# fankiat/sopht-mpi

Measured on NVIDIA B200. Metric: full_timestep_Mcell_updates_per_s, higher is better.
Workload: dtype f32

## Files before the change

sopht_mpi_b200/csrc/poisson_fft.cu:

```cuda
#include "fft_device.h"
#include "poisson.h"

#include <cstdlib>
#include <vector>

#define SB_P32_LINES(log2n) 8


#ifndef SB200_EMU
#define SB_DEV_ALLOC(ptr, bytes) (cudaMalloc((void**)&(ptr), (bytes)) == cudaSuccess)
#define SB_DEV_FREE(ptr) cudaFree(ptr)
#define SB_DEV_UPLOAD(dst, src, bytes, stream) \
  cudaMemcpyAsync(dst, src, bytes, cudaMemcpyHostToDevice, (cudaStream_t)(stream))
#define SB_STREAM_SYNC(stream) cudaStreamSynchronize((cudaStream_t)(stream))
#else
#define SB_DEV_ALLOC(ptr, bytes) (((ptr) = (decltype(ptr))malloc(bytes)) != nullptr)
#define SB_DEV_FREE(ptr) free(ptr)
#define SB_DEV_UPLOAD(dst, src, bytes, stream) memcpy(dst, src, bytes)
#define SB_STREAM_SYNC(stream) (void)0
#endif

struct SbLines {
  int inner, n1, n2;
  long long s1, s2;
  long long pt;
  int o1_shift = 30;
  long long s1_hi = 0;
  int gsh = 31;
  long long s_grp = 0;
  int rot = 0;
  SB_HD long long base(int i, int o1, int o2) const {
    return ((i + ((o1 >> 1) & rot)) & ((1u << gsh) - 1)) + (long long)(i >> gsh) * s_grp +
           (long long)(o1 & ((1 << o1_shift) - 1)) * s1 + (long long)(o1 >> o1_shift) * s1_hi + o2 * s2;
  }
};

template <typename T>
struct FieldRows {
  T* f;
  int ny, gs, dim;
  long long my, mx, vol;
  SB_D T* row(int c, int z, int y) const {
    return f + (dim == 3 ? c * vol + ((long long)(z + gs) * my + (y + gs)) * mx + gs
                         : c * vol + (long long)(y + gs) * mx + gs);
  }
  SB_D C2<T> load(int c, int z, int y, int m) const {
    const T* p = row(c, z, y) + 2 * m;
    if ((gs & 1) == 0) return *reinterpret_cast<const C2<T>*>(p);
    return C2<T>{p[0], p[1]};
  }
};
template <typename T>
struct GreensRows {
  SbGreens<T> g;
  int ny;
  SB_D C2<T> load(int, int z, int y, int m) const { return C2<T>{g(z, y, 2 * m), g(z, y, 2 * m + 1)}; }
};

static inline int sb_slab_kxl(int nx, int nranks) { return ((nx + 1 + nranks - 1) / nranks + 3) & ~3; }

struct SbRowBlocks {
  int kxl = 0;
  unsigned magic = 0;
  long long dblk = 0;
  SB_D long long rel(int k) const {
#ifdef SB200_EMU
    const int b = k / kxl;
#else
    const int b = (int)__umulhi((unsigned)k, magic);
#endif
    return (long long)b * dblk + k;
  }
  SB_D long long row(long long line, long long pitch) const { return line * (kxl ? (long long)kxl : pitch); }
};
static inline SbRowBlocks sb_row_blocks(int kxl, long long blk) {
  SbRowBlocks rb;
  rb.kxl = kxl;
  rb.magic = kxl ? (unsigned)((0x100000000ULL + (unsigned long long)kxl - 1) / (unsigned long long)kxl) : 0;
  rb.dblk = blk - kxl;
  return rb;
}

template <typename T, typename Rows, bool PRUNED, int LOG2N, int LINES>
__global__ void __launch_bounds__(LOG2N > 0 ? LINES * (1 << LOG2N) / SB_FFT_R : 512)
    sb_fft_x_r2c_kernel(SbFftPlan plan, int lines_rt, Rows rows, C2<T>* out, long long out_pitch,
                        const C2<T>* __restrict__ tw, const C2<T>* __restrict__ wpost, SbRowBlocks rb) {
  SB_DYN_SMEM(smem_raw);
  C2<T>* sm = reinterpret_cast<C2<T>*>(smem_raw);
  const int Tn = LOG2N > 0 ? (1 << LOG2N) / SB_FFT_R : plan.threads, N = LOG2N > 0 ? (1 << LOG2N) : plan.n;
  const int lines_per_block = LOG2N > 0 ? LINES : lines_rt;
  const int l = threadIdx.x / Tn, t = threadIdx.x - l * Tn;
  const int y = blockIdx.x * lines_per_block + l;
  const int z = blockIdx.y, c = blockIdx.z;
  const bool valid = y < rows.ny;
  const int yc = valid ? y : rows.ny - 1;
  const SbSmemLine<T, false> sl = sb_smem_line<T, false>(sm, l, 0, sb_fft_npad(N));
  constexpr int IN = PRUNED ? SB_FFT_R / 2 : SB_FFT_R;
  C2<T> v[SB_FFT_R];
#pragma unroll
  for (int p = 0; p < SB_FFT_R; ++p) v[p] = p < IN ? rows.load(c, z, yc, t + p * Tn) : C2<T>{T(0), T(0)};
  if constexpr (LOG2N > 0)
    sb_fft_forward_c<T, LOG2N, false, LINES>(v, t, tw, SbFftLineC<T, LOG2N, false, LINES>::line(sm, l));
  else
    sb_fft_forward<T, false>(v, plan, t, tw, sl);
#pragma unroll
  for (int p = 0; p < SB_FFT_R; ++p) sl.at(t + p * Tn) = v[p];
  __syncthreads();
  if (valid) {
    const long long line = ((long long)c * gridDim.y + z) * rows.ny + y;
    C2<T>* row = out + rb.row(line, out_pitch);
    C2<T> r[SB_FFT_R];
#pragma unroll
    for (int p = 0; p < SB_FFT_R; ++p) {
      const int k = t + p * Tn;
      const C2<T> zk = v[p];
      const C2<T> zc = cconj(sl.at((N - k) & (N - 1)));
      const C2<T> wd = cmul(wpost[k], csub(zk, zc));
      const C2<T> s = cadd(zk, zc);
      r[p] = C2<T>{T(0.5) * (s.x + wd.y), T(0.5) * (s.y - wd.x)};
    }
    const C2<T> last{v[0].x - v[0].y, T(0)};
    if (rb.kxl == 0) {
#pragma unroll
      for (int p = 0; p < SB_FFT_R; ++p) row[t + p * Tn] = r[p];
      if (t == 0) row[N] = last;
    } else {
#pragma unroll
      for (int p = 0; p < SB_FFT_R; ++p) row[rb.rel(t + p * Tn)] = r[p];
      if (t == 0) row[rb.rel(N)] = last;
    }
  }
}

template <typename T, int LOG2N, int LINES>
__global__ void __launch_bounds__(LOG2N > 0 ? LINES * (1 << LOG2N) / SB_FFT_R : 512)
    sb_fft_x_c2r_kernel(SbFftPlan plan, int lines_rt, const C2<T>* in, long long in_pitch,
                        FieldRows<T> rows, const C2<T>* __restrict__ tw, const C2<T>* __restrict__ wpost,
                        SbRowBlocks rb) {
  SB_DYN_SMEM(smem_raw);
  C2<T>* sm = reinterpret_cast<C2<T>*>(smem_raw);
  const int Tn = LOG2N > 0 ? (1 << LOG2N) / SB_FFT_R : plan.threads, N = LOG2N > 0 ? (1 << LOG2N) : plan.n;
  const int lines_per_block = LOG2N > 0 ? LINES : lines_rt;
  const int l = threadIdx.x / Tn, t = threadIdx.x - l * Tn;
  const int y = blockIdx.x * lines_per_block + l;
  const int z = blockIdx.y, c = blockIdx.z;
  const bool valid = y < rows.ny;
  const int yc = valid ? y : rows.ny - 1;
  const SbSmemLine<T, false> sl = sb_smem_line<T, false>(sm, l, 0, sb_fft_npad(N));
  const long long line = ((long long)c * gridDim.y + z) * rows.ny + yc;
  const C2<T>* row = in + rb.row(line, in_pitch);
  C2<T> v[SB_FFT_R];
  if (rb.kxl == 0) {
#pragma unroll
    for (int p = 0; p < SB_FFT_R; ++p) v[p] = row[t + p * Tn];
    if (t == 0) sl.at(N) = row[N];
  } else {
#pragma unroll
    for (int p = 0; p < SB_FFT_R; ++p) v[p] = row[rb.rel(t + p * Tn)];
    if (t == 0) sl.at(N) = row[rb.rel(N)];
  }
#pragma unroll
  for (int p = 0; p < SB_FFT_R; ++p) sl.at(t + p * Tn) = v[p];
  __syncthreads();
#pragma unroll
  for (int p = 0; p < SB_FFT_R; ++p) {
    const int k = t + p * Tn;
    const C2<T> xk = sl.at(k);
    const C2<T> xc = cconj(sl.at(N - k));
    const C2<T> wd = cmul(cconj(wpost[k]), csub(xk, xc));
    const C2<T> s = cadd(xk, xc);
    v[p] = C2<T>{s.x - wd.y, s.y + wd.x};
  }
  __syncthreads();
  if constexpr (LOG2N > 0)
    sb_fft_inverse_c<T, LOG2N, false, LINES>(v, t, tw, SbFftLineC<T, LOG2N, false, LINES>::line(sm, l));
  else
    sb_fft_inverse<T, false>(v, plan, t, tw, sl);
  if (valid) {
    T* orow = rows.row(c, z, y);
#pragma unroll
    for (int p = 0; p < SB_FFT_R / 2; ++p) {
      const int m = t + p * Tn;
      if ((rows.gs & 1) == 0) {
        *reinterpret_cast<C2<T>*>(orow + 2 * m) = v[p];
      } else {
        orow[2 * m] = v[p].x;
        orow[2 * m + 1] = v[p].y;
      }
    }
  }
}

constexpr int sb_lb_threads(int log2n, int lines) { return log2n > 0 ? lines * ((1 << log2n) / SB_FFT_R) : 512; }
constexpr int sb_lb_blocks(int log2n, int lines, size_t elem) {
  return (log2n > 0 && elem == 4) ? 1024 / sb_lb_threads(log2n, lines) : 1;
}

constexpr int sb_lb_blocks_conv(int log2n, int lines, size_t elem) {
  if (!(log2n > 0 && elem == 4)) return 1;
  const int nt = sb_lb_threads(log2n, lines);
  return nt <= 256 ? 768 / nt : nt <= 512 ? 1024 / nt : 1;
}

template <typename T>
struct SbGreensTable {
  const T* g;
  long long g_pt, g_s1;
  int n1_full = 1;
  int o1_off = 0;
  const T* g2 = nullptr;
  int kx0 = 0, kx_last = 1 << 30;
};

SB_D void sb_cp_async16(void* smem_dst, const void* gsrc) {
#ifdef SB200_EMU
  memcpy(smem_dst, gsrc, 16);
#else
  asm volatile("cp.async.cg.shared.global [%0], [%1], 16;" ::"r"((unsigned)__cvta_generic_to_shared(smem_dst)),
               "l"(gsrc)
               : "memory");
#endif
}
SB_D void sb_cp_async_wait_all() {
#ifndef SB200_EMU
  asm volatile("cp.async.wait_all;" ::: "memory");
#endif
}

template <typename T, int MODE, int LOG2N, int LINES, bool G2>
__global__ void __launch_bounds__(sb_lb_threads(LOG2N, LINES), MODE == 1 ? sb_lb_blocks_conv(LOG2N, LINES, sizeof(T)) : sb_lb_blocks(LOG2N, LINES, sizeof(T)))
    sb_fft_strided_kernel(SbFftPlan plan, int lb_shift_rt, const C2<T>* in, SbLines lin, C2<T>* out, SbLines lout,
                          const C2<T>* __restrict__ tw, SbGreensTable<T> gt) {
  SB_DYN_SMEM(smem_raw);
  C2<T>* sm = reinterpret_cast<C2<T>*>(smem_raw);
  const int Tn = LOG2N > 0 ? (1 << LOG2N) / SB_FFT_R : plan.threads, n = LOG2N > 0 ? (1 << LOG2N) : plan.n;
  constexpr int LINES_SHIFT = LINES == 16 ? 4 : LINES == 8 ? 3 : LINES == 4 ? 2 : LINES == 2 ? 1 : 0;
  const int lb_shift = LOG2N > 0 ? LINES_SHIFT : lb_shift_rt;
  const int l = threadIdx.x & ((1 << lb_shift) - 1), t = threadIdx.x >> lb_shift;
  static_assert(!G2 || (MODE == 1 && LOG2N > 0 && sizeof(T) == 4), "thread-order table: fused float kernel");
  const int ib = G2 ? blockIdx.y : blockIdx.x;
  const int i = (ib << lb_shift) + l;
  const int o1 = G2 ? blockIdx.z : blockIdx.y, o2 = G2 ? blockIdx.x : blockIdx.z;
  const bool valid = i < lin.inner;
  const int ic = valid ? i : lin.inner - 1;
  const SbSmemLine<T, true> sl = sb_smem_line<T, true>(sm, l, lb_shift, sb_fft_npad(n));
  float4* gstage = nullptr;
  if constexpr (G2) {
    constexpr int NT = LINES * ((1 << LOG2N) / SB_FFT_R);
    gstage = reinterpret_cast<float4*>(sm + LINES * SbFftC<LOG2N>::npad) + threadIdx.x;
    const int g1 = o1 + gt.o1_off;
    const int m1 = g1 <= (gt.n1_full >> 1) ? g1 : gt.n1_full - g1;
    const float4* src = reinterpret_cast<const float4*>(gt.g2) +
                        (((long long)m1 * gridDim.y + ib) * NT + threadIdx.x) * 4;
#pragma unroll
    for (int k = 0; k < 4; ++k) sb_cp_async16(gstage + k * NT, src + k);
  }
  constexpr int IN = (MODE == 0 || MODE == 1) ? SB_FFT_R / 2 : SB_FFT_R;
  constexpr int OUT = (MODE == 1 || MODE == 2) ? SB_FFT_R / 2 : SB_FFT_R;
  C2<T> v[SB_FFT_R];
  {
    const C2<T>* gp = in + lin.base(ic, o1, o2);
    const long long sp = (long long)Tn * lin.pt;
    gp += (long long)t * lin.pt;
#pragma unroll
    for (int p = 0; p < SB_FFT_R; ++p) {
      if (p < IN) {
        v[p] = *gp;
        gp += sp;
      } else {
        v[p] = C2<T>{T(0), T(0)};
      }
    }
  }
  if constexpr (MODE != 2) {
    if constexpr (LOG2N > 0)
      sb_fft_forward_c<T, LOG2N, true, LINES>(v, t, tw, SbFftLineC<T, LOG2N, true, LINES>::line(sm, l));
    else
      sb_fft_forward<T, true>(v, plan, t, tw, sl);
  }
  if constexpr (G2) {
    constexpr int NT = LINES * ((1 << LOG2N) / SB_FFT_R);
    sb_cp_async_wait_all();
#pragma unroll
    for (int k = 0; k < 4; ++k) {
      const float4 gv = gstage[k * NT];
      v[4 * k] = cscale(v[4 * k], gv.x);
      v[4 * k + 1] = cscale(v[4 * k + 1], gv.y);
      v[4 * k + 2] = cscale(v[4 * k + 2], gv.z);
      v[4 * k + 3] = cscale(v[4 * k + 3], gv.w);
    }
  } else if constexpr (MODE == 1) {
    const int g1 = o1 + gt.o1_off;
    const int m1 = g1 <= (gt.n1_full >> 1) ? g1 : gt.n1_full - g1;
    const int kxg = ic + gt.kx0 < gt.kx_last ? ic + gt.kx0 : gt.kx_last;
    const T* g = gt.g + ((long long)m1 * gt.g_s1 + kxg);
    const long long gs = (long long)Tn * gt.g_pt;
    const T* ga = g + (long long)t * gt.g_pt;
    const T* gb = g + (long long)(n - t - (SB_FFT_R / 2) * Tn) * gt.g_pt;
#pragma unroll
    for (int p = 0; p < SB_FFT_R / 2; ++p) {
      v[p] = cscale(v[p], *ga);
      v[p + SB_FFT_R / 2] = cscale(v[p + SB_FFT_R / 2], *gb);
      ga += gs;
      gb -= gs;
    }
  }
  if constexpr (MODE == 1 || MODE == 2) {
    if constexpr (LOG2N > 0)
      sb_fft_inverse_c<T, LOG2N, true, LINES>(v, t, tw, SbFftLineC<T, LOG2N, true, LINES>::line(sm, l));
    else
      sb_fft_inverse<T, true>(v, plan, t, tw, sl);
  }
  if (valid) {
    C2<T>* gp = out + lout.base(i, o1, o2);
    const long long sp = (long long)Tn * lout.pt;
    gp += (long long)t * lout.pt;
#pragma unroll
    for (int p = 0; p < OUT; ++p) {
      *gp = v[p];
      gp += sp;
    }
  }
}

constexpr int sb_p32_min_blocks(int log2n, int lines) {
  const int nt = lines * ((1 << log2n) / SB_FFT_P32);
  return 512 / nt > 0 ? 512 / nt : 1;
}

template <typename T, int MODE, int LOG2N, int LINES>
__global__ void __launch_bounds__(LINES*((1 << LOG2N) / SB_FFT_P32), sb_p32_min_blocks(LOG2N, LINES))
    sb_fft_strided32_kernel(const C2<T>* in, SbLines lin, C2<T>* out, SbLines lout,
                            const C2<T>* __restrict__ tw, SbGreensTable<T> gt) {
  SB_DYN_SMEM(smem_raw);
  using FC = SbFft32C<LOG2N>;
  constexpr int PT = SB_FFT_P32, Tn = FC::Tn;
  constexpr int LINES_SHIFT = LINES == 16 ? 4 : LINES == 8 ? 3 : LINES == 4 ? 2 : LINES == 2 ? 1 : 0;
  constexpr int IN = (MODE == 0 || MODE == 1) ? PT / 2 : PT;
  constexpr int OUT = (MODE == 1 || MODE == 2) ? PT / 2 : PT;
  C2<T>* sm = reinterpret_cast<C2<T>*>(smem_raw);
  const int l = threadIdx.x & (LINES - 1), t = threadIdx.x >> LINES_SHIFT;
  const int i = (blockIdx.x << LINES_SHIFT) + l;
  const int o1 = blockIdx.y, o2 = blockIdx.z;
  const bool valid = i < lin.inner;
  const int ic = valid ? i : lin.inner - 1;
  C2<T>* sline = sm + l;
  C2<T> v[PT];
  {
    const C2<T>* gp = in + lin.base(ic, o1, o2);
    const long long sp = (long long)Tn * lin.pt;
    gp += (long long)t * lin.pt;
#pragma unroll
    for (int p = 0; p < PT; ++p) {
      if (p < IN) {
        v[p] = *gp;
        gp += sp;
      } else {
        v[p] = C2<T>{T(0), T(0)};
      }
    }
  }
  if constexpr (MODE != 2) sb_fft32_forward_c<T, LOG2N, LINES, MODE == 1>(v, t, tw, sline);
  if constexpr (MODE == 1) {
    const int g1 = o1 + gt.o1_off;
    const int m1 = g1 <= (gt.n1_full >> 1) ? g1 : gt.n1_full - g1;
    const int kxg = ic + gt.kx0 < gt.kx_last ? ic + gt.kx0 : gt.kx_last;
    const T* g = gt.g + ((long long)m1 * gt.g_s1 + kxg);
    const long long gs = (long long)Tn * gt.g_pt;
    const T* ga = g + (long long)t * gt.g_pt;
    const T* gb = g + (long long)(FC::n - t - (PT / 2) * Tn) * gt.g_pt;
#pragma unroll
    for (int p = 0; p < PT / 2; ++p) {
      v[p] = cscale(v[p], *ga);
      v[p + PT / 2] = cscale(v[p + PT / 2], *gb);
      ga += gs;
      gb -= gs;
    }
  }
  if constexpr (MODE == 1 || MODE == 2) sb_fft32_inverse_c<T, LOG2N, LINES, false>(v, t, tw, sline);
  if (valid) {
    C2<T>* gp = out + lout.base(i, o1, o2);
    const long long sp = (long long)Tn * lout.pt;
    gp += (long long)t * lout.pt;
#pragma unroll
    for (int p = 0; p < OUT; ++p) {
      *gp = v[p];
      gp += sp;
    }
  }
}

#ifndef SB200_EMU
SB_D unsigned sb_smem_u32(const void* p) { return (unsigned)__cvta_generic_to_shared(p); }
SB_D void sb_mbar_init(unsigned long long* bar, unsigned count) {
  asm volatile("mbarrier.init.shared::cta.b64 [%0], %1;" ::"r"(sb_smem_u32(bar)), "r"(count) : "memory");
  asm volatile("fence.mbarrier_init.release.cluster;" ::: "memory");
}
SB_D void sb_bulk_load(void* smem_dst, const void* gsrc, unsigned bytes, unsigned long long* bar) {
  asm volatile("fence.proxy.async.shared::cta;" ::: "memory");
  asm volatile("mbarrier.arrive.expect_tx.shared::cta.b64 _, [%0], %1;" ::"r"(sb_smem_u32(bar)), "r"(bytes)
               : "memory");
  asm volatile("cp.async.bulk.shared::cluster.global.mbarrier::complete_tx::bytes [%0], [%1], %2, [%3];" ::"r"(
                   sb_smem_u32(smem_dst)),
               "l"(gsrc), "r"(bytes), "r"(sb_smem_u32(bar))
               : "memory");
}
SB_D void sb_mbar_wait_warp(unsigned long long* bar, unsigned parity) {
  unsigned ok;
  do {
    asm volatile(
        "{\n.reg .pred p;\nmbarrier.try_wait.parity.shared::cta.b64 p, [%1], %2;\nselp.u32 %0, 1, 0, p;\n}"
        : "=r"(ok)
        : "r"(sb_smem_u32(bar)), "r"(parity)
        : "memory");
  } while (!__all_sync(0xffffffffu, ok));
}
SB_D void sb_mbar_expect_if(bool pred, unsigned long long* bar, unsigned bytes) {
  asm volatile(
      "{\n.reg .pred p;\nsetp.ne.u32 p, %0, 0;\n"
      "@p fence.proxy.async.shared::cta;\n"
      "@p mbarrier.arrive.expect_tx.shared::cta.b64 _, [%2], %1;\n}" ::"r"((unsigned)pred),
      "r"(bytes), "r"(sb_smem_u32(bar))
      : "memory");
}
SB_D void sb_bulk_copy_if(bool pred, void* smem_dst, const void* gsrc, unsigned bytes, unsigned long long* bar) {
  asm volatile(
      "{\n.reg .pred p;\nsetp.ne.u32 p, %0, 0;\n"
      "@p cp.async.bulk.shared::cluster.global.mbarrier::complete_tx::bytes [%1], [%2], %3, [%4];\n}" ::"r"(
          (unsigned)pred),
      "r"(sb_smem_u32(smem_dst)), "l"(gsrc), "r"(bytes), "r"(sb_smem_u32(bar))
      : "memory");
}
SB_D void sb_mbar_arrive(unsigned long long* bar) {
  asm volatile("mbarrier.arrive.shared::cta.b64 _, [%0];" ::"r"(sb_smem_u32(bar)) : "memory");
}
SB_D void sb_fence_async_smem() { asm volatile("fence.proxy.async.shared::cta;" ::: "memory"); }
SB_D void sb_bulk_store(void* gdst, const void* smem_src, unsigned bytes) {
  asm volatile("cp.async.bulk.global.shared::cta.bulk_group [%0], [%1], %2;" ::"l"(gdst), "r"(sb_smem_u32(smem_src)),
               "r"(bytes)
               : "memory");
  asm volatile("cp.async.bulk.commit_group;" ::: "memory");
}
SB_D void sb_bulk_wait_read() { asm volatile("cp.async.bulk.wait_group.read 0;" ::: "memory"); }
SB_D void sb_bulk_wait_all() { asm volatile("cp.async.bulk.wait_group 0;" ::: "memory"); }
#else
SB_D void sb_mbar_init(unsigned long long* bar, unsigned count) {
  __atomic_store_n(bar, ((unsigned long long)count << 8) | count, __ATOMIC_SEQ_CST);
}
SB_D void sb_mbar_update(unsigned long long* bar, unsigned arrivals, long long tx16) {
  unsigned long long e = __atomic_load_n(bar, __ATOMIC_SEQ_CST);
  for (;;) {
    const unsigned long long cnt = (e >> 8) & 0xffu, pend = (e & 0xffu) - arrivals;
    const unsigned long long tx = (unsigned long long)((long long)((e >> 16) & 0xffffu) + tx16) & 0xffffu;
    unsigned long long d = (e & 0xffffffff00000000ULL) | (tx << 16) | (cnt << 8) | pend;
    if (pend == 0 && tx == 0) d = (((e >> 32) + 1) << 32) | (cnt << 8) | cnt;
    if (__atomic_compare_exchange_n(bar, &e, d, false, __ATOMIC_SEQ_CST, __ATOMIC_SEQ_CST)) return;
  }
}
SB_D void sb_mbar_arrive(unsigned long long* bar) { sb_mbar_update(bar, 1, 0); }
SB_D void sb_mbar_expect_if(bool pred, unsigned long long* bar, unsigned bytes) {
  if (pred) sb_mbar_update(bar, 1, bytes / 16);
}
SB_D void sb_bulk_copy_if(bool pred, void* smem_dst, const void* gsrc, unsigned bytes, unsigned long long* bar) {
  if (!pred) return;
  memcpy(smem_dst, gsrc, bytes);
  sb_mbar_update(bar, 0, -(long long)(bytes / 16));
}
SB_D void sb_bulk_load(void* smem_dst, const void* gsrc, unsigned bytes, unsigned long long* bar) {
  sb_mbar_expect_if(true, bar, bytes);
  sb_bulk_copy_if(true, smem_dst, gsrc, bytes, bar);
}
SB_D void sb_mbar_wait_warp(unsigned long long* bar, unsigned parity) {
  while (((__atomic_load_n(bar, __ATOMIC_SEQ_CST) >> 32) & 1u) == parity) std::this_thread::yield();
}
SB_D void sb_fence_async_smem() { __atomic_thread_fence(__ATOMIC_SEQ_CST); }
SB_D void sb_bulk_store(void* gdst, const void* smem_src, unsigned bytes) { memcpy(gdst, smem_src, bytes); }
SB_D void sb_bulk_wait_read() {}
SB_D void sb_bulk_wait_all() {}
#endif

template <int LOG2N>
struct SbZw {
  using FC = SbFft32C<LOG2N>;
  static constexpr int Tn = FC::Tn, LINES = 8, NT = LINES * Tn, NW = NT / 32, NZ = FC::n / 2;
  static constexpr unsigned TILE = NZ * LINES;
  static constexpr int XL = SbFft32W<LOG2N>::XL;
  static constexpr int BLOCKS = LOG2N >= 10 ? 2 : 4;
  static constexpr size_t smem = 2 * TILE * sizeof(C2<float>) + (size_t)LINES * XL * sizeof(float) + 128;
  static_assert((2 + NW) * 8 + 2 * 4 + 2 * 4 <= 128, "barriers, arrival counters, tile ids");
};

template <int LOG2N>
__global__ void __launch_bounds__(SbZw<LOG2N>::NT, SbZw<LOG2N>::BLOCKS)
    sb_fft_zconvw_kernel(C2<float>* B, int ntiles, int ncomp, int ng, int nky, const C2<float>* __restrict__ tw,
                         const float* __restrict__ g5, int n1_full, int* next_tile) {
  using Z = SbZw<LOG2N>;
  constexpr int PT = SB_FFT_P32, Tn = Z::Tn, N = Z::FC::n;
  constexpr unsigned TILE = Z::TILE, TILE_BYTES = TILE * sizeof(C2<float>);
  SB_DYN_SMEM(smem_raw);
  C2<float>* tbuf = reinterpret_cast<C2<float>*>(smem_raw);
  float* xch = reinterpret_cast<float*>(tbuf + 2 * TILE);
  unsigned long long* bars = reinterpret_cast<unsigned long long*>(xch + Z::LINES * Z::XL);
  unsigned* cnt = reinterpret_cast<unsigned*>(bars + 2 + Z::NW);
  int* tile_of = reinterpret_cast<int*>(cnt + 2);
  const int tid = threadIdx.x, l = tid / Tn, t = tid % Tn, lane = tid & 31, warp = tid >> 5;
  float* xl = xch + l * Z::XL;
  const int slot = (l + (t >> 1)) & 7;
  auto tile_offset = [&](int tile) {
    const int c = tile % ncomp, r = tile / ncomp;
    return (((long long)c * ng + r % ng) * nky + r / ng) * (long long)TILE;
  };
  auto arm = [&](int b) {
    const int tile = atomicAdd(next_tile, 1);
    tile_of[b] = tile;
    if (tile < ntiles)
      sb_bulk_load(tbuf + b * TILE, B + tile_offset(tile), TILE_BYTES, bars + b);
    else
      sb_mbar_arrive(bars + b);
  };
  if (tid == 0) {
    sb_mbar_init(bars + 0, 1);
    sb_mbar_init(bars + 1, 1);
    for (int w = 0; w < Z::NW; ++w) sb_mbar_init(bars + 2 + w, 1);
    cnt[0] = cnt[1] = 0;
  }
  __syncthreads();
  if (tid == 0) {
    arm(0);
    arm(1);
  }
  for (int k = 0;; ++k) {
    const int b = k & 1;
    C2<float>* tb = tbuf + b * TILE + slot;
    sb_mbar_wait_warp(bars + b, (unsigned)(k >> 1) & 1u);
    if (tile_of[b] >= ntiles) break;
    C2<float> v[PT];
#pragma unroll
    for (int p = 0; p < PT / 2; ++p) v[p] = tb[(t + p * Tn) * Z::LINES];
    sb_fft32w_forward<LOG2N, true>(v, t, tw, xl);
    __syncwarp();
    {
      const int r = tile_of[b] / ncomp, kxg = r % ng, ky = r / ng;
      const int m1 = ky <= (n1_full >> 1) ? ky : n1_full - ky;
      constexpr int LW = 32 / Tn;
      const float* src = g5 + (((long long)m1 * ng + kxg) * Z::LINES + warp * LW) * N;
      sb_mbar_expect_if(lane == 0, bars + 2 + warp, LW * N * sizeof(float));
#pragma unroll
      for (int i = 0; i < LW; ++i)
        sb_bulk_copy_if(lane == 0, xch + (warp * LW + i) * Z::XL, src + i * N, N * sizeof(float), bars + 2 + warp);
    }
    sb_fft32w_second<LOG2N>(v, t, tw);
    sb_mbar_wait_warp(bars + 2 + warp, (unsigned)k & 1u);
#pragma unroll
    for (int p = 0; p < PT; ++p) v[p] = cscale_conj(v[p], xl[t + p * Tn]);
    sb_fft32w_forward<LOG2N, false>(v, t, tw, xl);
    sb_fft32w_second<LOG2N>(v, t, tw);
#pragma unroll
    for (int p = 0; p < PT / 2; ++p) tb[(t + p * Tn) * Z::LINES] = C2<float>{v[p].x, -v[p].y};
    sb_fence_async_smem();
    __syncwarp();
    if (lane == 0) {
      __threadfence_block();
      if ((atomicAdd(cnt + b, 1u) + 1) % Z::NW == 0) {
        __threadfence_block();
        sb_bulk_store(B + tile_offset(tile_of[b]), tbuf + b * TILE, TILE_BYTES);
        sb_bulk_wait_read();
        arm(b);
      }
    }
  }
  if (lane == 0) sb_bulk_wait_all();
}

template <typename T>
struct GreensExtractOp {
  T* g;
  const C2<T>* full;
  long long pitch, n2y, hy1;
  T scale;
  SB_D void operator()(long long i) const {
    const long long kx = i % pitch, r = i / pitch;
    const long long ky = r % hy1, kz = r / hy1;
    g[i] = full[(kz * n2y + ky) * pitch + kx].x * scale;
  }
};

template <typename T>
struct GreensThreadOrderOp {
  T* g2;
  const T* g;
  long long g_pt, g_s1;
  int n, Tn, lines, nib, pitch;
  int kx0, inner;
  int warp_order = 0;
  SB_D void operator()(long long idx) const {
    int p, l, t;
    long long r;
    if (warp_order) {
      const int k = (int)(idx % n), mk = k <= (n >> 1) ? k : n - k;
      r = idx / n;
      l = (int)(r % lines);
      r /= lines;
      const int ib = (int)(r % nib), i = ib * lines + l, kx = kx0 + i;
      const long long m1 = r / nib;
      g2[idx] = (i < inner && kx < pitch) ? g[mk * g_pt + m1 * g_s1 + kx] : T(0);
      return;
    } else {
      p = (int)(idx % SB_FFT_R);
      r = idx / SB_FFT_R;
      l = (int)(r % lines);
      r /= lines;
      t = (int)(r % Tn);
      r /= Tn;
    }
    const int ib = (int)(r % nib);
    const long long m1 = r / nib;
    const int k = t + p * Tn, mk = k <= (n >> 1) ? k : n - k, i = ib * lines + l, kx = kx0 + i;
    g2[idx] = (i < inner && kx < pitch) ? g[mk * g_pt + m1 * g_s1 + kx] : T(0);
  }
};

template <typename T>
struct SbFftState {
  SbFftPlan px, py, pz;
  C2<T>*twx = nullptr, *twy = nullptr, *twz = nullptr, *wpost = nullptr;
  C2<T>* A = nullptr;
  C2<T>* B = nullptr;
  T* G = nullptr;
  T* G2 = nullptr;
  long long P = 0;
  size_t bytes = 0;
  int kxl = 0;
  bool zconv = false;
  int ng = 0;
  int* tile_counter = nullptr;
  bool profile = false, have_times = false;
#ifndef SB200_EMU
  cudaEvent_t ev[6] = {nullptr, nullptr, nullptr, nullptr, nullptr, nullptr};
#endif
  void mark(int i, void* stream) {
#ifndef SB200_EMU
    if (profile) cudaEventRecord(ev[i], (cudaStream_t)stream);
#else
    (void)i; (void)stream;
#endif
  }
};

template <typename T>
static C2<T>* make_twiddles(int n, int count, double denom, void* stream) {
  std::vector<C2<T>> h(count);
  for (int k = 0; k < count; ++k) {
    const double a = -2.0 * M_PI * (double)k / denom;
    h[k] = C2<T>{(T)std::cos(a), (T)std::sin(a)};
  }
  C2<T>* d = nullptr;
  if (!SB_DEV_ALLOC(d, sizeof(C2<T>) * count)) return nullptr;
  SB_DEV_UPLOAD(d, h.data(), sizeof(C2<T>) * count, stream);
  SB_STREAM_SYNC(stream);
  (void)n;
  return d;
}

static int lines_per_block_for(int threads_per_line, size_t elem, bool strided) {
  int lb = strided ? (elem == 4 ? 8 : 4) : 1;
  while (lb * threads_per_line < 128) lb *= 2;
  while (lb > 1 && lb * threads_per_line > 512) lb /= 2;
  return lb;
}

template <typename T>
constexpr int sb_strided_lines(int log2n, int mode) {
  (void)mode;
  return (sizeof(T) == 4 && log2n <= 10) ? 8 : 4;
}
constexpr int sb_xpass_lines(int log2n) { return log2n <= 7 ? 16 : log2n == 8 ? 8 : log2n == 9 ? 4 : log2n == 10 ? 2 : 1; }

template <typename T, typename Rows, bool PRUNED, int LOG2N>
static int launch_x_r2c_c(const SbFftPlan& plan, int ny, int nz, int ncomp, const Rows& rows, C2<T>* out,
                          long long pitch, const C2<T>* tw, const C2<T>* wpost, void* stream,
                          const SbRowBlocks& rb) {
  constexpr int LINES = LOG2N > 0 ? sb_xpass_lines(LOG2N) : 0;
  const int lb = LOG2N > 0 ? LINES : lines_per_block_for(plan.threads, sizeof(T), false);
  const size_t smem = (size_t)lb * sb_fft_npad(plan.n) * sizeof(C2<T>);
  SB_KERNEL_ATTR_SMEM((sb_fft_x_r2c_kernel<T, Rows, PRUNED, LOG2N, LINES>), smem);
  const dim3 grid((unsigned)((ny + lb - 1) / lb), (unsigned)nz, (unsigned)ncomp);
  SB_LAUNCH_COOP((sb_fft_x_r2c_kernel<T, Rows, PRUNED, LOG2N, LINES>), grid, dim3(lb * plan.threads), smem,
                 stream, plan, lb, rows, out, pitch, tw, wpost, rb);
  SB_CHECK_LAUNCH("fft_x_r2c");
  return 0;
}
template <typename T, typename Rows, bool PRUNED>
static int launch_x_r2c(const SbFftPlan& plan, int ny, int nz, int ncomp, const Rows& rows, C2<T>* out,
                        long long pitch, const C2<T>* tw, const C2<T>* wpost, void* stream,
                        const SbRowBlocks& rb = SbRowBlocks()) {
  if constexpr (PRUNED) {
    switch (plan.log2n) {
      case 8: return launch_x_r2c_c<T, Rows, PRUNED, 8>(plan, ny, nz, ncomp, rows, out, pitch, tw, wpost, stream, rb);
      case 9: return launch_x_r2c_c<T, Rows, PRUNED, 9>(plan, ny, nz, ncomp, rows, out, pitch, tw, wpost, stream, rb);
      case 10: return launch_x_r2c_c<T, Rows, PRUNED, 10>(plan, ny, nz, ncomp, rows, out, pitch, tw, wpost, stream, rb);
      default: break;
    }
  }
  return launch_x_r2c_c<T, Rows, PRUNED, 0>(plan, ny, nz, ncomp, rows, out, pitch, tw, wpost, stream, rb);
}

template <typename T, int LOG2N>
static int launch_x_c2r_c(const SbFftPlan& plan, int ny, int nz, int ncomp, const C2<T>* in, long long pitch,
                          const FieldRows<T>& dst, const C2<T>* tw, const C2<T>* wpost, void* stream,
                          const SbRowBlocks& rb) {
  constexpr int LINES = LOG2N > 0 ? sb_xpass_lines(LOG2N) : 0;
  const int lb = LOG2N > 0 ? LINES : lines_per_block_for(plan.threads, sizeof(T), false);
  const size_t smem = (size_t)lb * sb_fft_npad(plan.n) * sizeof(C2<T>);
  SB_KERNEL_ATTR_SMEM((sb_fft_x_c2r_kernel<T, LOG2N, LINES>), smem);
  const dim3 grid((unsigned)((ny + lb - 1) / lb), (unsigned)nz, (unsigned)ncomp);
  SB_LAUNCH_COOP((sb_fft_x_c2r_kernel<T, LOG2N, LINES>), grid, dim3(lb * plan.threads), smem, stream, plan, lb,
                 in, pitch, dst, tw, wpost, rb);
  SB_CHECK_LAUNCH("fft_x_c2r");
  return 0;
}
template <typename T>
static int launch_x_c2r(const SbFftPlan& plan, int ny, int nz, int ncomp, const C2<T>* in, long long pitch,
                        const FieldRows<T>& dst, const C2<T>* tw, const C2<T>* wpost, void* stream,
                        const SbRowBlocks& rb = SbRowBlocks()) {
  {
    switch (plan.log2n) {
      case 8: return launch_x_c2r_c<T, 8>(plan, ny, nz, ncomp, in, pitch, dst, tw, wpost, stream, rb);
      case 9: return launch_x_c2r_c<T, 9>(plan, ny, nz, ncomp, in, pitch, dst, tw, wpost, stream, rb);
      case 10: return launch_x_c2r_c<T, 10>(plan, ny, nz, ncomp, in, pitch, dst, tw, wpost, stream, rb);
      default: break;
    }
  }
  return launch_x_c2r_c<T, 0>(plan, ny, nz, ncomp, in, pitch, dst, tw, wpost, stream, rb);
}

constexpr bool sb_use_p32(int mode, int log2n) {
  return (log2n == 10 && mode <= 2) || (log2n == 9 && mode <= 1);
}

template <typename T, int MODE, int LOG2N>
static int launch_strided32(const C2<T>* in, const SbLines& lin, C2<T>* out, const SbLines& lout,
                            const C2<T>* tw, const SbGreensTable<T>& gt, void* stream) {
  constexpr int LINES = SB_P32_LINES(LOG2N), NT = LINES * ((1 << LOG2N) / SB_FFT_P32);
  const size_t smem = sizeof(C2<T>) * (size_t)LINES * SbFft32C<LOG2N>::npad;
  const dim3 grid((unsigned)((lin.inner + LINES - 1) / LINES), (unsigned)lin.n1, (unsigned)lin.n2);
  SB_KERNEL_ATTR_SMEM((sb_fft_strided32_kernel<T, MODE, LOG2N, LINES>), smem);
  SB_LAUNCH_COOP((sb_fft_strided32_kernel<T, MODE, LOG2N, LINES>), grid, dim3(NT), smem, stream, in, lin, out, lout,
                 tw, gt);
  SB_CHECK_LAUNCH("fft_strided32");
  return 0;
}

template <typename T, int MODE, int LOG2N>
static int launch_strided_c(const SbFftPlan& plan, const C2<T>* in, const SbLines& lin, C2<T>* out,
                            const SbLines& lout, const C2<T>* tw, const SbGreensTable<T>& gt, void* stream) {
  constexpr int LINES = LOG2N > 0 ? sb_strided_lines<T>(LOG2N, MODE) : 0;
  if constexpr (sizeof(T) == 4 && sb_use_p32(MODE, LOG2N)) {
    return launch_strided32<T, MODE, LOG2N>(in, lin, out, lout, tw, gt, stream);
  } else {
    const int lb = LOG2N > 0 ? LINES : lines_per_block_for(plan.threads, sizeof(T), true);
    const size_t smem = (size_t)lb * sb_fft_npad(plan.n) * sizeof(C2<T>);
    int lb_shift = 0;
    while ((1 << lb_shift) < lb) ++lb_shift;
    const unsigned nib = (unsigned)((lin.inner + lb - 1) / lb);
    if constexpr (MODE == 1 && LOG2N > 0 && sizeof(T) == 4) {
      if (gt.g2) {
        const size_t smem2 = smem + (size_t)lb * plan.threads * 64;
        const dim3 grid2((unsigned)lin.n2, nib, (unsigned)lin.n1);
        SB_KERNEL_ATTR_SMEM((sb_fft_strided_kernel<T, MODE, LOG2N, LINES, true>), smem2);
        SB_LAUNCH_COOP((sb_fft_strided_kernel<T, MODE, LOG2N, LINES, true>), grid2, dim3(lb * plan.threads), smem2,
                       stream, plan, lb_shift, in, lin, out, lout, tw, gt);
        SB_CHECK_LAUNCH("fft_strided");
        return 0;
      }
    }
    const dim3 grid(nib, (unsigned)lin.n1, (unsigned)lin.n2);
    SB_KERNEL_ATTR_SMEM((sb_fft_strided_kernel<T, MODE, LOG2N, LINES, false>), smem);
    SB_LAUNCH_COOP((sb_fft_strided_kernel<T, MODE, LOG2N, LINES, false>), grid, dim3(lb * plan.threads), smem, stream,
                   plan, lb_shift, in, lin, out, lout, tw, gt);
    SB_CHECK_LAUNCH("fft_strided");
    return 0;
  }
}
template <typename T, int MODE>
static int launch_strided(const SbFftPlan& plan, const C2<T>* in, const SbLines& lin, C2<T>* out,
                          const SbLines& lout, const C2<T>* tw, const SbGreensTable<T>& gt, void* stream) {
  if constexpr (MODE != 3) {
    switch (plan.log2n) {
      case 8: return launch_strided_c<T, MODE, 8>(plan, in, lin, out, lout, tw, gt, stream);
      case 9: return launch_strided_c<T, MODE, 9>(plan, in, lin, out, lout, tw, gt, stream);
      case 10: return launch_strided_c<T, MODE, 10>(plan, in, lin, out, lout, tw, gt, stream);
      case 11:
        if constexpr (sizeof(T) == 4) return launch_strided_c<T, MODE, 11>(plan, in, lin, out, lout, tw, gt, stream);
        break;
      default: break;
    }
  }
  return launch_strided_c<T, MODE, 0>(plan, in, lin, out, lout, tw, gt, stream);
}

template <int LOG2N>
static int launch_zconvw(C2<float>* B, int ncomp, int ng, int nky, const C2<float>* tw, const float* g3,
                         int n1_full, int* tile_counter, void* stream) {
  using Z = SbZw<LOG2N>;
  SB_REQUIRE(tile_counter != nullptr, "fft_zconvw: no tile counter");
  sb_memset_async(tile_counter, 0, sizeof(int), stream);
  SB_KERNEL_ATTR_SMEM((sb_fft_zconvw_kernel<LOG2N>), Z::smem);
  const long long ntiles = (long long)ncomp * ng * nky;
  long long resident = 148LL * Z::BLOCKS;
#ifndef SB200_EMU
  {
    static int sms = 0, per_sm = 0;
    if (sms == 0) {
      int dev = 0;
      cudaGetDevice(&dev);
      cudaDeviceGetAttribute(&sms, cudaDevAttrMultiProcessorCount, dev);
      cudaOccupancyMaxActiveBlocksPerMultiprocessor(&per_sm, sb_fft_zconvw_kernel<LOG2N>, Z::NT, Z::smem);
      if (per_sm < 1) per_sm = 1;
    }
    resident = (long long)sms * per_sm;
  }
#else
  resident = 3;
#endif
  const unsigned grid = (unsigned)(ntiles < resident ? ntiles : resident);
  SB_LAUNCH_COOP((sb_fft_zconvw_kernel<LOG2N>), dim3(grid), dim3(Z::NT), Z::smem, stream, B, (int)ntiles, ncomp, ng,
                 nky, tw, g3, n1_full, tile_counter);
  SB_CHECK_LAUNCH("fft_zconvw");
  return 0;
}
template <typename T>
static int launch_zconv(int log2n, C2<T>* B, int ncomp, int ng, int nky, const C2<T>* tw, const T* g2, int n1_full,
                        int* tile_counter, void* stream) {
  if constexpr (sizeof(T) == 4) {
    if (log2n == 9) return launch_zconvw<9>(B, ncomp, ng, nky, tw, g2, n1_full, tile_counter, stream);
    if (log2n == 10) return launch_zconvw<10>(B, ncomp, ng, nky, tw, g2, n1_full, tile_counter, stream);
  }
  sb_set_error("fft_zconv: unsupported transform length");
  return -1;
}

template <typename T>
static int fft_create_t(sb200_poisson* p, void* stream) {
  auto* st = new SbFftState<T>();
  p->backend_state = st;
  const int nz = p->nz, ny = p->ny, nx = p->nx;
  SB_REQUIRE(sb_fft_make_plan(nx, &st->px) == 0 && sb_fft_make_plan(2 * ny, &st->py) == 0 &&
                 (p->dim == 2 || sb_fft_make_plan(2 * nz, &st->pz) == 0),
             "fft backend needs power-of-two grid sizes (nx >= 16, ny >= 8, nz >= 8)");
  SB_REQUIRE(nx <= 4096 && ny <= 2048 && nz <= 2048, "fft backend: grid too large for one line per block");
  st->P = nx + 2;
  const long long P = st->P;
  st->twx = make_twiddles<T>(nx, nx, (double)nx, stream);
  st->wpost = make_twiddles<T>(nx, nx, 2.0 * nx, stream);
  st->twy = make_twiddles<T>(2 * ny, 2 * ny, 2.0 * ny, stream);
  if (p->dim == 3) st->twz = make_twiddles<T>(2 * nz, 2 * nz, 2.0 * nz, stream);
  SB_REQUIRE(st->twx && st->wpost && st->twy && (p->dim == 2 || st->twz), "fft backend: twiddle allocation");
  if (p->nranks > 1) {
    SB_REQUIRE(p->dim == 3, "fft backend: slab decomposition is implemented for 3D grids");
    SB_REQUIRE(p->nranks == 2 || p->nranks == 4 || p->nranks == 8,
               "fft backend: slab decomposition needs 2, 4 or 8 ranks");
    SB_REQUIRE(nz % p->nranks == 0 && nz / p->nranks >= 2 * p->gs, "fft backend: nz must split into slabs");
  }
  st->kxl = p->nranks > 1 ? sb_slab_kxl(nx, p->nranks) : 0;
  const size_t a_bytes = p->nranks == 1 ? sizeof(C2<T>) * 3 * (size_t)(p->dim == 3 ? nz : 1) * ny * P : 0;
  {
    const int inner = p->nranks > 1 ? st->kxl : nx + 1;
    st->ng = (inner + 7) / 8;
    st->zconv = sizeof(T) == 4 && p->dim == 3 && (st->pz.log2n == 9 || st->pz.log2n == 10);
  }
  if (st->zconv) SB_REQUIRE(SB_DEV_ALLOC(st->tile_counter, 64), "fft backend: cannot allocate the tile counter");
  const size_t b_bytes = p->dim != 3 ? 0
                         : st->zconv ? sizeof(C2<T>) * 3 * (size_t)nz * 2 * ny * 8 * st->ng
                         : p->nranks == 1 ? sizeof(C2<T>) * 3 * (size_t)nz * 2 * ny * P
                                          : sizeof(C2<T>) * 3 * (size_t)nz * 2 * ny * st->kxl;
  const size_t g_bytes = sizeof(T) * (p->dim == 3 ? (nz + 1) : 1) * (ny + 1) * P;
  if (a_bytes) SB_REQUIRE(SB_DEV_ALLOC(st->A, a_bytes), "fft backend: cannot allocate x-pass buffer");
  if (b_bytes) SB_REQUIRE(SB_DEV_ALLOC(st->B, b_bytes), "fft backend: cannot allocate y-pass buffer");
  if (b_bytes && st->zconv) sb_memset_async(st->B, 0, b_bytes, stream);
  SB_REQUIRE(SB_DEV_ALLOC(st->G, g_bytes), "fft backend: cannot allocate Green's table");
  st->bytes = a_bytes + b_bytes + g_bytes;

  const long long n2z = p->dim == 3 ? 2LL * nz : 1, n2y = 2LL * ny;
  C2<T>* full = nullptr;
  SB_REQUIRE(SB_DEV_ALLOC(full, sizeof(C2<T>) * n2z * n2y * P), "fft backend: cannot allocate Green's scratch");
  GreensRows<T> gl;
  void* lines_dev = nullptr;
  int e = sb_poisson_make_greens<T>(p, &gl.g, &lines_dev, stream);
  if (e) return e;
  gl.ny = (int)n2y;
  if ((e = launch_x_r2c<T, GreensRows<T>, false>(st->px, (int)n2y, (int)n2z, 1, gl, full, P, st->twx, st->wpost,
                                                 stream)))
    return e;
  SbGreensTable<T> none{nullptr, 0, 0};
  {
    SbLines ly{nx + 1, (int)n2z, 1, n2y * P, 0, P};
    if ((e = launch_strided<T, 3>(st->py, full, ly, full, ly, st->twy, none, stream))) return e;
  }
  if (p->dim == 3) {
    SbLines lz{nx + 1, (int)n2y, 1, P, 0, n2y * P};
    if ((e = launch_strided<T, 3>(st->pz, full, lz, full, lz, st->twz, none, stream))) return e;
  }
  double dxp = 1.0;
  for (int d = 0; d < p->dim; ++d) dxp *= p->dx;
  const double scale = dxp / ((double)n2z * (double)n2y * 2.0 * (double)nx);
  const long long hz1 = p->dim == 3 ? nz + 1 : 1;
  e = sb_launch_flat(hz1 * (ny + 1) * P, GreensExtractOp<T>{st->G, full, P, n2y, (long long)ny + 1, (T)scale},
                     stream, "greens_extract");
  if constexpr (sizeof(T) == 4) {
    if (!e && p->dim == 3 && st->pz.log2n >= 8 && st->pz.log2n <= 11) {
      const int lines = st->zconv ? SB_P32_LINES(st->pz.log2n) : sb_strided_lines<T>(st->pz.log2n, 1);
      const int inner = p->nranks > 1 ? st->kxl : nx + 1, kx0 = p->nranks > 1 ? p->rank * st->kxl : 0;
      const int nib = (inner + lines - 1) / lines;
      const long long count = (long long)(ny + 1) * nib * lines * 2 * nz;
      SB_REQUIRE(SB_DEV_ALLOC(st->G2, sizeof(T) * count), "fft backend: cannot allocate the thread-order table");
      st->bytes += sizeof(T) * count;
      e = sb_launch_flat(count, GreensThreadOrderOp<T>{st->G2, st->G, (long long)(ny + 1) * P, P, 2 * nz,
                                                       2 * nz / SB_FFT_R, lines, nib, (int)P, kx0, inner, st->zconv},
                         stream, "greens_thread_order");
    }
  }
  SB_STREAM_SYNC(stream);
  sb_poisson_free_greens_lines(lines_dev);
  SB_DEV_FREE(full);
  return e;
}

template <typename T>
static int fft_solve_t(sb200_poisson* p, void* solution, const void* rhs, int ncomp, void* stream) {
  auto* st = (SbFftState<T>*)p->backend_state;
  SB_REQUIRE(ncomp >= 1 && ncomp <= 3, "poisson_solve: ncomp must be 1..3");
  const int nz = p->dim == 3 ? p->nz : 1, ny = p->ny, nx = p->nx, gs = p->gs;
  const long long P = st->P;
  const long long my = ny + 2 * gs, mx = nx + 2 * gs;
  const long long vol = (p->dim == 3 ? nz + 2LL * gs : 1) * my * mx;
  int e;
  FieldRows<T> src{(T*)rhs, ny, gs, p->dim, my, mx, vol};
  st->mark(0, stream);
  if ((e = launch_x_r2c<T, FieldRows<T>, true>(st->px, ny, nz, ncomp, src, st->A, P, st->twx, st->wpost, stream)))
    return e;
  st->mark(1, stream);
  SbGreensTable<T> none{nullptr, 0, 0};
  if (p->dim == 3) {
    if (st->zconv) {
      const long long NZ = nz, NKY = 2LL * ny, tile = NZ * 8;
      SbLines la{nx + 1, nz, ncomp, (long long)ny * P, (long long)nz * ny * P, P};
      SbLines lb{nx + 1, nz, ncomp, 8, (long long)st->ng * NKY * tile, tile};
      lb.gsh = 3;
      lb.s_grp = NKY * tile;
      lb.rot = 7;
      if ((e = launch_strided<T, 0>(st->py, st->A, la, st->B, lb, st->twy, none, stream))) return e;
      st->mark(2, stream);
      if ((e = launch_zconv<T>(st->pz.log2n, st->B, ncomp, st->ng, (int)NKY, st->twz, st->G2, 2 * ny, st->tile_counter, stream))) return e;
      st->mark(3, stream);
      if ((e = launch_strided<T, 2>(st->py, st->B, lb, st->A, la, st->twy, none, stream))) return e;
      st->mark(4, stream);
    } else {
      const long long cstride = 2LL * nz * ny * P;
      SbLines la{nx + 1, nz, ncomp, (long long)ny * P, (long long)nz * ny * P, P};
      SbLines lb{nx + 1, nz, ncomp, 2LL * ny * P, cstride, P};
      if ((e = launch_strided<T, 0>(st->py, st->A, la, st->B, lb, st->twy, none, stream))) return e;
      st->mark(2, stream);
      SbLines lz{nx + 1, 2 * ny, ncomp, P, cstride, 2LL * ny * P};
      SbGreensTable<T> gt{st->G, (long long)(ny + 1) * P, P, 2 * ny, 0};
      gt.g2 = st->G2;
      if ((e = launch_strided<T, 1>(st->pz, st->B, lz, st->B, lz, st->twz, gt, stream))) return e;
      st->mark(3, stream);
      if ((e = launch_strided<T, 2>(st->py, st->B, lb, st->A, la, st->twy, none, stream))) return e;
      st->mark(4, stream);
    }
  } else {
    st->mark(2, stream);
    SbLines ly{nx + 1, 1, ncomp, 0, (long long)ny * P, P};
    SbGreensTable<T> gt{st->G, P, 0, 1, 0};
    if ((e = launch_strided<T, 1>(st->py, st->A, ly, st->A, ly, st->twy, gt, stream))) return e;
    st->mark(3, stream);
    st->mark(4, stream);
  }
  FieldRows<T> dst{(T*)solution, ny, gs, p->dim, my, mx, vol};
  e = launch_x_c2r<T>(st->px, ny, nz, ncomp, (const C2<T>*)st->A, P, dst, (const C2<T>*)st->twx,
                      (const C2<T>*)st->wpost, stream);
  st->mark(5, stream);
  st->have_times = st->profile && e == 0;
  return e;
}

template <typename T>
static int fft_set_profiling_t(sb200_poisson* p, int enable) {
  auto* st = (SbFftState<T>*)p->backend_state;
#ifndef SB200_EMU
  if (enable && !st->ev[0])
    for (auto& ev : st->ev) SB_REQUIRE(cudaEventCreate(&ev) == cudaSuccess, "poisson profiling: cudaEventCreate");
#endif
  st->profile = enable != 0;
  st->have_times = false;
  return 0;
}
template <typename T>
static int fft_last_stage_ms_t(sb200_poisson* p, float* ms_out, int n) {
  auto* st = (SbFftState<T>*)p->backend_state;
  SB_REQUIRE(st->have_times, "poisson profiling: no profiled solve yet");
  for (int i = 0; i < n && i < 5; ++i) {
#ifndef SB200_EMU
    if (i == 0) SB_REQUIRE(cudaEventSynchronize(st->ev[5]) == cudaSuccess, "poisson profiling: event sync");
    SB_REQUIRE(cudaEventElapsedTime(&ms_out[i], st->ev[i], st->ev[i + 1]) == cudaSuccess,
               "poisson profiling: elapsed time");
#else
    ms_out[i] = 0.f;
#endif
  }
  return 0;
}
extern "C" int sb200_poisson_set_profiling(sb200_poisson_t* p, int enable) {
  SB_REQUIRE(p && p->backend == 1 && p->backend_state && p->nranks == 1,
             "poisson profiling needs a single-rank handle of the fft backend");
  SB_DISPATCH_DTYPE(p->dtype, return fft_set_profiling_t<T>(p, enable));
}
extern "C" int sb200_poisson_last_stage_ms(sb200_poisson_t* p, float* ms_out, int n) {
  SB_REQUIRE(p && p->backend == 1 && p->backend_state && ms_out && n >= 1,
             "poisson profiling needs a handle of the fft backend");
  SB_DISPATCH_DTYPE(p->dtype, return fft_last_stage_ms_t<T>(p, ms_out, n));
}
// ... 137 lines not shown
```

Measured before the change: 9489.

## Use warp-shuffle 32-point FFT kernels for x-pass r2c/c2r at n=512,1024

Adds specialized float x-direction real-to-complex and complex-to-real kernels for log2n 9 and 10. They build on the register-resident sb_fft32w routines and do the real-FFT post/pre twiddle pairing with warp shuffles, so the shared-memory round trip used by the generic per-line kernel is dropped. Each block handles more lines with a small scratch area and launch bounds of 2 blocks. The risks are higher register pressure and the correctness of the partner-lane index math, including the wraparound handled by lane t==0.

```diff
diff --git a/sopht_mpi_b200/csrc/poisson_fft.cu b/sopht_mpi_b200/csrc/poisson_fft.cu
--- a/sopht_mpi_b200/csrc/poisson_fft.cu
+++ b/sopht_mpi_b200/csrc/poisson_fft.cu
@@ -186,6 +186,112 @@
       } else {
         orow[2 * m] = v[p].x;
         orow[2 * m + 1] = v[p].y;
+      }
+    }
+  }
+}
+
+template <int LOG2N>
+struct SbXw {
+  using FC = SbFft32C<LOG2N>;
+  static constexpr int Tn = FC::Tn, N = FC::n, LINES = 8 * 32 / Tn, NT = LINES * Tn;
+  static constexpr int XL = SbFft32W<LOG2N>::XL;
+  static constexpr size_t smem = (size_t)LINES * XL * sizeof(float);
+};
+SB_D int sb_xw_partner(int lane, int t, int Tn) { return (lane - t) | ((Tn - t) & (Tn - 1)); }
+
+template <typename Rows, int LOG2N>
+__global__ void __launch_bounds__(SbXw<LOG2N>::NT, 2)
+    sb_fft_x_r2c_w_kernel(Rows rows, C2<float>* out, long long out_pitch, const C2<float>* __restrict__ tw,
+                          const C2<float>* __restrict__ wpost, SbRowBlocks rb) {
+  using X = SbXw<LOG2N>;
+  constexpr int PT = SB_FFT_P32, Tn = X::Tn, N = X::N;
+  SB_DYN_SMEM(smem_raw);
+  const int tid = threadIdx.x, l = tid / Tn, t = tid % Tn, lane = tid & 31;
+  const int y = blockIdx.x * X::LINES + l, z = blockIdx.y, c = blockIdx.z;
+  const bool valid = y < rows.ny;
+  const int yc = valid ? y : rows.ny - 1;
+  float* xl = reinterpret_cast<float*>(smem_raw) + l * X::XL;
+  C2<float> v[PT];
+#pragma unroll
+  for (int p = 0; p < PT / 2; ++p) v[p] = rows.load(c, z, yc, t + p * Tn);
+  sb_fft32w_forward<LOG2N, true>(v, t, tw, xl);
+  sb_fft32w_second<LOG2N>(v, t, tw);
+  const int src = sb_xw_partner(lane, t, Tn);
+  C2<float>* row = out + rb.row(((long long)c * gridDim.y + z) * rows.ny + yc, out_pitch);
+  const bool blocked = rb.kxl != 0;
+  auto offset = [&](int k) { return blocked ? rb.rel(k) : (long long)k; };
+#pragma unroll
+  for (int p = 0; p < PT; ++p) {
+    const C2<float> zp{__shfl_sync(0xffffffffu, v[PT - 1 - p].x, src), __shfl_sync(0xffffffffu, v[PT - 1 - p].y, src)};
+    const C2<float> zc = cconj(t == 0 ? v[(PT - p) & (PT - 1)] : zp);
+    const int k = t + p * Tn;
+    const C2<float> zk = v[p];
+    const C2<float> wd = cmul(wpost[k], csub(zk, zc));
+    const C2<float> s = cadd(zk, zc);
+    C2<float>* dst = row + offset(k);
+    const C2<float> r{0.5f * (s.x + wd.y), 0.5f * (s.y - wd.x)};
+    if (valid) *dst = r;
+  }
+  if (valid && t == 0) row[offset(N)] = C2<float>{v[0].x - v[0].y, 0.f};
+}
+
+template <int LOG2N>
+__global__ void __launch_bounds__(SbXw<LOG2N>::NT, 2)
+    sb_fft_x_c2r_w_kernel(const C2<float>* in, long long in_pitch, FieldRows<float> rows,
+                          const C2<float>* __restrict__ tw, const C2<float>* __restrict__ wpost, SbRowBlocks rb) {
+  using X = SbXw<LOG2N>;
+  constexpr int PT = SB_FFT_P32, Tn = X::Tn, N = X::N;
+  SB_DYN_SMEM(smem_raw);
+  const int tid = threadIdx.x, l = tid / Tn, t = tid % Tn, lane = tid & 31;
+  const int y = blockIdx.x * X::LINES + l, z = blockIdx.y, c = blockIdx.z;
+  const bool valid = y < rows.ny;
+  const int yc = valid ? y : rows.ny - 1;
+  float* xl = reinterpret_cast<float*>(smem_raw) + l * X::XL;
+  const C2<float>* row = in + rb.row(((long long)c * gridDim.y + z) * rows.ny + yc, in_pitch);
+  C2<float> v[PT], xn;
+  if (rb.kxl == 0) {
+#pragma unroll
+    for (int p = 0; p < PT; ++p) v[p] = row[t + p * Tn];
+    xn = row[N];
+  } else {
+#pragma unroll
+    for (int p = 0; p < PT; ++p) v[p] = row[rb.rel(t + p * Tn)];
+    xn = row[rb.rel(N)];
+  }
+  const int src = sb_xw_partner(lane, t, Tn);
+  C2<float> carry = xn;
+  auto pre = [&](C2<float> xk, C2<float> xm, int k) {
+    const C2<float> xc = cconj(xm);
+    const C2<float> wd = cmul(cconj(wpost[k]), csub(xk, xc));
+    const C2<float> s = cadd(xk, xc);
+    return C2<float>{s.x - wd.y, -(s.y + wd.x)};
+  };
+#pragma unroll
+  for (int j = 0; j < PT / 2; ++j) {
+    const C2<float> a = v[j], b = v[PT - 1 - j];
+    C2<float> ma{__shfl_sync(0xffffffffu, b.x, src), __shfl_sync(0xffffffffu, b.y, src)};
+    C2<float> mb{__shfl_sync(0xffffffffu, a.x, src), __shfl_sync(0xffffffffu, a.y, src)};
+    if (t == 0) {
+      ma = carry;
+      mb = j == PT / 2 - 1 ? b : v[j + 1];
+    }
+    carry = b;
+    v[j] = pre(a, ma, t + j * Tn);
+    v[PT - 1 - j] = pre(b, mb, t + (PT - 1 - j) * Tn);
+  }
+  sb_fft32w_forward<LOG2N, false>(v, t, tw, xl);
+  sb_fft32w_second<LOG2N>(v, t, tw);
+  if (valid) {
+    float* orow = rows.row(c, z, y);
+#pragma unroll
+    for (int p = 0; p < PT / 2; ++p) {
+      const int m = t + p * Tn;
+      if ((rows.gs & 1) == 0) {
+        *reinterpret_cast<C2<float>*>(orow + 2 * m) = C2<float>{v[p].x, -v[p].y};
+      } else {
+        orow[2 * m] = v[p].x;
+        orow[2 * m + 1] = -v[p].y;
       }
     }
   }
@@ -676,19 +782,31 @@
 }
 constexpr int sb_xpass_lines(int log2n) { return log2n <= 7 ? 16 : log2n == 8 ? 8 : log2n == 9 ? 4 : log2n == 10 ? 2 : 1; }
 
+constexpr bool sb_use_xw(size_t elem, int log2n) { return elem == 4 && (log2n == 9 || log2n == 10); }
+
 template <typename T, typename Rows, bool PRUNED, int LOG2N>
 static int launch_x_r2c_c(const SbFftPlan& plan, int ny, int nz, int ncomp, const Rows& rows, C2<T>* out,
                           long long pitch, const C2<T>* tw, const C2<T>* wpost, void* stream,
                           const SbRowBlocks& rb) {
-  constexpr int LINES = LOG2N > 0 ? sb_xpass_lines(LOG2N) : 0;
-  const int lb = LOG2N > 0 ? LINES : lines_per_block_for(plan.threads, sizeof(T), false);
-  const size_t smem = (size_t)lb * sb_fft_npad(plan.n) * sizeof(C2<T>);
-  SB_KERNEL_ATTR_SMEM((sb_fft_x_r2c_kernel<T, Rows, PRUNED, LOG2N, LINES>), smem);
-  const dim3 grid((unsigned)((ny + lb - 1) / lb), (unsigned)nz, (unsigned)ncomp);
-  SB_LAUNCH_COOP((sb_fft_x_r2c_kernel<T, Rows, PRUNED, LOG2N, LINES>), grid, dim3(lb * plan.threads), smem,
-                 stream, plan, lb, rows, out, pitch, tw, wpost, rb);
-  SB_CHECK_LAUNCH("fft_x_r2c");
-  return 0;
+  if constexpr (PRUNED && sb_use_xw(sizeof(T), LOG2N)) {
+    using X = SbXw<LOG2N>;
+    SB_KERNEL_ATTR_SMEM((sb_fft_x_r2c_w_kernel<Rows, LOG2N>), X::smem);
+    const dim3 grid((unsigned)((ny + X::LINES - 1) / X::LINES), (unsigned)nz, (unsigned)ncomp);
+    SB_LAUNCH_COOP((sb_fft_x_r2c_w_kernel<Rows, LOG2N>), grid, dim3(X::NT), X::smem, stream, rows, out, pitch, tw,
+                   wpost, rb);
+    SB_CHECK_LAUNCH("fft_x_r2c");
+    return 0;
+  } else {
+    constexpr int LINES = LOG2N > 0 ? sb_xpass_lines(LOG2N) : 0;
+    const int lb = LOG2N > 0 ? LINES : lines_per_block_for(plan.threads, sizeof(T), false);
+    const size_t smem = (size_t)lb * sb_fft_npad(plan.n) * sizeof(C2<T>);
+    SB_KERNEL_ATTR_SMEM((sb_fft_x_r2c_kernel<T, Rows, PRUNED, LOG2N, LINES>), smem);
+    const dim3 grid((unsigned)((ny + lb - 1) / lb), (unsigned)nz, (unsigned)ncomp);
+    SB_LAUNCH_COOP((sb_fft_x_r2c_kernel<T, Rows, PRUNED, LOG2N, LINES>), grid, dim3(lb * plan.threads), smem,
+                   stream, plan, lb, rows, out, pitch, tw, wpost, rb);
+    SB_CHECK_LAUNCH("fft_x_r2c");
+    return 0;
+  }
 }
 template <typename T, typename Rows, bool PRUNED>
 static int launch_x_r2c(const SbFftPlan& plan, int ny, int nz, int ncomp, const Rows& rows, C2<T>* out,
@@ -709,15 +827,24 @@
 static int launch_x_c2r_c(const SbFftPlan& plan, int ny, int nz, int ncomp, const C2<T>* in, long long pitch,
                           const FieldRows<T>& dst, const C2<T>* tw, const C2<T>* wpost, void* stream,
                           const SbRowBlocks& rb) {
-  constexpr int LINES = LOG2N > 0 ? sb_xpass_lines(LOG2N) : 0;
-  const int lb = LOG2N > 0 ? LINES : lines_per_block_for(plan.threads, sizeof(T), false);
-  const size_t smem = (size_t)lb * sb_fft_npad(plan.n) * sizeof(C2<T>);
-  SB_KERNEL_ATTR_SMEM((sb_fft_x_c2r_kernel<T, LOG2N, LINES>), smem);
-  const dim3 grid((unsigned)((ny + lb - 1) / lb), (unsigned)nz, (unsigned)ncomp);
-  SB_LAUNCH_COOP((sb_fft_x_c2r_kernel<T, LOG2N, LINES>), grid, dim3(lb * plan.threads), smem, stream, plan, lb,
-                 in, pitch, dst, tw, wpost, rb);
-  SB_CHECK_LAUNCH("fft_x_c2r");
-  return 0;
+  if constexpr (sb_use_xw(sizeof(T), LOG2N)) {
+    using X = SbXw<LOG2N>;
+    SB_KERNEL_ATTR_SMEM((sb_fft_x_c2r_w_kernel<LOG2N>), X::smem);
+    const dim3 grid((unsigned)((ny + X::LINES - 1) / X::LINES), (unsigned)nz, (unsigned)ncomp);
+    SB_LAUNCH_COOP((sb_fft_x_c2r_w_kernel<LOG2N>), grid, dim3(X::NT), X::smem, stream, in, pitch, dst, tw, wpost, rb);
+    SB_CHECK_LAUNCH("fft_x_c2r");
+    return 0;
+  } else {
+    constexpr int LINES = LOG2N > 0 ? sb_xpass_lines(LOG2N) : 0;
+    const int lb = LOG2N > 0 ? LINES : lines_per_block_for(plan.threads, sizeof(T), false);
+    const size_t smem = (size_t)lb * sb_fft_npad(plan.n) * sizeof(C2<T>);
+    SB_KERNEL_ATTR_SMEM((sb_fft_x_c2r_kernel<T, LOG2N, LINES>), smem);
+    const dim3 grid((unsigned)((ny + lb - 1) / lb), (unsigned)nz, (unsigned)ncomp);
+    SB_LAUNCH_COOP((sb_fft_x_c2r_kernel<T, LOG2N, LINES>), grid, dim3(lb * plan.threads), smem, stream, plan, lb,
+                   in, pitch, dst, tw, wpost, rb);
+    SB_CHECK_LAUNCH("fft_x_c2r");
+    return 0;
+  }
 }
 template <typename T>
 static int launch_x_c2r(const SbFftPlan& plan, int ny, int nz, int ncomp, const C2<T>* in, long long pitch,
```

Result: faster. 9700 (median of 6 runs) (+2.2%).
